# bwfbowen/muax

Hardware: AMD Instinct MI355X
Metric: batched act() env-steps/sec at num_simulations=50 (higher is better)
Workload: dtype f32; 1 GPU; cartpole: 4096 roots/GPU, obs 4, MLP embed 8, A=2, support 10, num_simulations=50, dirichlet 0.25/0.3, tiebreak=threefry, temperature 1; roots_per_gpu=4096, num_simulations=50, parallelism=roots sharded x1, no collective, backend=none (one rank), launcher=none

## Files before the change

### muax_amd/csrc/mz_act.hip

```cpp
#include <hip/hip_runtime.h>

#include <cstdlib>
#include <cstring>

#include "mz_handle.h"
#include "mz_fused_launch.h"
#include "mz_wide_launch.h"

using mzh::fail;

template <class Call>
static int dispatch_with_scratch(mzs_handle* h, mz::FusedParams& p, int* rc, Call call) {
  const size_t BN = (size_t)h->cfg.batch * (h->cfg.num_simulations + 1);
  *rc = call();
  for (int tries = 0; tries < 2 && (*rc == mz::kNeedEmbScratch || *rc >= mz::kNeedPathScratch); ++tries) {
    if (*rc == mz::kNeedEmbScratch) {
      MZS_HIP(h, hipMalloc(reinterpret_cast<void**>(&h->fused_emb), BN * h->cfg.embed_dim * sizeof(float)));
      p.emb_scratch = h->fused_emb;
    } else {
      const int words = *rc - mz::kNeedPathScratch;
      if (h->fused_path) MZS_HIP(h, hipFree(h->fused_path));
      h->fused_path = nullptr;
      h->fused_path_words = 0;
      MZS_HIP(h, hipMalloc(reinterpret_cast<void**>(&h->fused_path), BN * words * sizeof(int32_t)));
      h->fused_path_words = words;
      p.path_scratch = h->fused_path;
      p.path_words = words;
    }
    *rc = call();
  }
  return MZS_OK;
}

extern "C" {

int mzs_act_mlp(mzs_handle* h, const mzs_act_args* a, void* stream_) {
  if (!h) return MZS_E_INVALID;
  if (!a || a->struct_size != (int32_t)sizeof(mzs_act_args))
    return fail(h, MZS_E_INVALID, "mzs_act_mlp: null or size mismatch (ABI)");
  if (!h->have_weights) return fail(h, MZS_E_INVALID, "mzs_act_mlp: call mzs_mlp_set_weights first");
  if (!a->obs || !a->action || !a->action_weights || !a->root_value)
    return fail(h, MZS_E_INVALID, "mzs_act_mlp: obs/action/action_weights/root_value must be set");
  const mzs_config& c = h->cfg;
  if (c.policy == 0 && !a->dirichlet_noise && a->dirichlet_fraction != 0.0f)
    return fail(h, MZS_E_INVALID, "mzs_act_mlp: dirichlet_fraction != 0 needs dirichlet_noise");
  if (c.num_simulations > mz::kMaxSims) {
    if (h->allow_generic) return mzh::act_mlp_generic(h, a, stream_);
    return fail(h, MZS_E_UNSUPPORTED, "mzs_act_mlp: no fused kernel instance for num_simulations > 256; use the generic route "
                                      "(mzs_mlp_allow_generic) or the step-wise path");
  }
  hipStream_t stream = static_cast<hipStream_t>(stream_);
  MZS_HIP(h, hipSetDevice(c.device));

  mz::FusedParams p;
  memset(&p, 0, sizeof p);
  p.obs = a->obs; p.dirichlet_noise = a->dirichlet_noise; p.invalid = a->invalid_actions; p.gumbel = a->gumbel;
  const mzs_mlp_weights& w = h->w;
  mzh::copy_weights(w, p);
  p.action = a->action; p.action_weights = a->action_weights; p.root_value = a->root_value;
  p.search_value = a->search_value; p.depth_sum = a->depth_sum;
  if (a->tree) {
    const mzs_tree_view& t = *a->tree;
    const void* const* tp = reinterpret_cast<const void* const*>(&t);
    for (int i = 0; i < 12; ++i)
      if (!tp[i]) return fail(h, MZS_E_INVALID, "mzs_act_mlp: tree view has a null array");
    p.t_node_visits = t.node_visits; p.t_raw_values = t.raw_values; p.t_node_values = t.node_values;
    p.t_parents = t.parents; p.t_action_from_parent = t.action_from_parent;
    p.t_children_index = t.children_index; p.t_children_prior_logits = t.children_prior_logits;
    p.t_children_values = t.children_values; p.t_children_visits = t.children_visits;
    p.t_children_rewards = t.children_rewards; p.t_children_discounts = t.children_discounts;
    p.t_embeddings = t.embeddings;
    p.export_tree = 1;
  }
  p.B = c.batch; p.obs_dim = w.obs_dim; p.S = c.num_simulations; p.max_depth = c.max_depth;
  p.support = w.support_size; p.pred_on_parent = w.recurrent_pred_on;
  p.pb_c_init = c.pb_c_init; p.pb_c_base = c.pb_c_base;
  p.dirichlet_fraction = a->dirichlet_fraction; p.discount = w.discount; p.temperature = a->temperature;
  p.global_batch = (uint64_t)c.global_batch; p.root_offset = (uint64_t)c.root_offset;
  p.prof = h->prof;
  p.emb_scratch = p.export_tree ? nullptr : h->fused_emb;
  if (c.policy == 1) {
    if (!h->fused_table) {
      const std::vector<int32_t> table = mzh::visit_table(c.max_num_considered_actions, c.num_simulations);
      MZS_HIP(h, hipMalloc(reinterpret_cast<void**>(&h->fused_table), table.size() * sizeof(int32_t)));
      MZS_HIP(h, hipMemcpy(h->fused_table, table.data(), table.size() * sizeof(int32_t), hipMemcpyHostToDevice));
    }
    p.visit_table = h->fused_table;
    p.max_considered = c.max_num_considered_actions;
    p.gumbel_scale = c.gumbel_scale;
    mzh::h_split(a->key, 2, 1, p.k_gumbel);
  }
  mzh::derive_keys(a->key, h->cfg.num_simulations, h->k_sample, h->sim_keys.data());
  p.k_sample[0] = h->k_sample[0]; p.k_sample[1] = h->k_sample[1];
  memcpy(p.sim_keys, h->sim_keys.data(), sizeof(uint32_t) * 2 * (size_t)c.num_simulations);

  const int A = c.num_actions, E = c.embed_dim, F = 2 * w.support_size + 1, N = c.num_simulations + 1;
  p.F = F;
  const int mode = c.policy == 1 ? (c.qtransform == 1 ? 3 : 2) : (c.tiebreak ? 1 : 0);
  std::vector<mz::FusedDispatch> groups = {mz::fused_dispatch_g0, mz::fused_dispatch_g1, mz::fused_dispatch_g2,
                                           mz::fused_dispatch_g3, mz::fused_dispatch_g4};
  mz::jit_dispatchers(mode, &groups);
  if (h->allow_generic && getenv("MZS_FORCE_GENERIC") != nullptr) return mzh::act_mlp_generic(h, a, stream_);
  for (int compact = (c.batch > 16 * h->cu_count) ? 1 : 0; compact >= 0; --compact) {
    p.path_scratch = h->fused_path;
    p.path_words = h->fused_path_words;
    for (size_t gi = 0; gi < groups.size(); ++gi) {
      std::string err;
      int rc = 0;
      auto call = [&] { return groups[gi](mode, c.device, p, stream, A, E, F, N, compact != 0, &err); };
      if (int e = dispatch_with_scratch(h, p, &rc, call)) return e;
      if (rc == mz::kNoFusedInstance) continue;
      if (rc != MZS_OK) return fail(h, rc, "mzs_act_mlp: %s", err.c_str());
      return MZS_OK;
    }
  }
  if (mode >= 2 ? h->allow_wide_gumbel : h->allow_wide) {
    std::string err;
    int rc = 0;
    auto call = [&] { return mz::wide_dispatch(mode, h->allow_wide_gumbel, c.device, p, stream, A, E, F, &err); };
    if (int e = dispatch_with_scratch(h, p, &rc, call)) return e;
    if (rc == MZS_OK) return MZS_OK;
    if (rc != mz::kNoFusedInstance) return fail(h, rc, "mzs_act_mlp: %s", err.c_str());
  }
  if (h->allow_generic) return mzh::act_mlp_generic(h, a, stream_);
  return fail(h, MZS_E_UNSUPPORTED,
              "mzs_act_mlp: no fused kernel instance for this (A, E, F, S) (muax_amd/csrc/mz_instances.def); use the step-wise path");
}

int mzs_act_mlp_host(mzs_handle* h, const mzs_act_host_args* a, void* stream_) {
  if (!h) return MZS_E_INVALID;
  if (!a || a->struct_size != (int32_t)sizeof(mzs_act_host_args))
    return fail(h, MZS_E_INVALID, "mzs_act_mlp_host: null or size mismatch (ABI)");
  if (!h->have_weights) return fail(h, MZS_E_INVALID, "mzs_act_mlp_host: call mzs_mlp_set_weights first");
  if (!a->obs || !a->action || !a->action_weights || !a->root_value)
    return fail(h, MZS_E_INVALID, "mzs_act_mlp_host: obs/action/action_weights/root_value must be set");
  const mzs_config& c = h->cfg;
  hipStream_t stream = static_cast<hipStream_t>(stream_);
  MZS_HIP(h, hipSetDevice(c.device));
  const size_t B = (size_t)c.batch, A = (size_t)c.num_actions, OD = (size_t)h->w.obs_dim;
  const size_t obs_b = B * OD * 4, noise_b = B * A * 4, inv_b = (B * A + 3) / 4 * 4, in_b = obs_b + noise_b + inv_b;
  const size_t out_b = B * (2 + A) * 4;
  if (h->host_in_bytes < in_b) {
    if (h->host_in) { hipHostFree(h->host_in); h->host_in = nullptr; }
    MZS_HIP(h, hipHostMalloc(&h->host_in, in_b, hipHostMallocDefault));
    h->host_in_bytes = in_b;
  }
  if (!h->host_out) MZS_HIP(h, hipHostMalloc(&h->host_out, out_b, hipHostMallocDefault));
  if (!h->dev_noise) MZS_HIP(h, hipMalloc(&h->dev_noise, noise_b));
  char* hin = static_cast<char*>(h->host_in);
  char* hin_dev = nullptr;
  float* hout_dev = nullptr;
  MZS_HIP(h, hipHostGetDevicePointer(reinterpret_cast<void**>(&hin_dev), h->host_in, 0));
  MZS_HIP(h, hipHostGetDevicePointer(reinterpret_cast<void**>(&hout_dev), h->host_out, 0));
  const bool muzero = c.policy == 0;
  const bool given = muzero && a->dirichlet_noise != nullptr;
  const bool draw = muzero && !given && a->draw_dirichlet != 0 && a->dirichlet_fraction != 0.0f;
  float* d_noise = static_cast<float*>(h->dev_noise);
  if (draw) {
    uint32_t kd[2];
    mzh::h_split(a->key, 3, 1, kd);
    if (int rc = mzs_dirichlet(c.device, kd, a->dirichlet_alpha, c.batch, c.num_actions, c.global_batch, c.root_offset,
                               d_noise, stream_))
      return fail(h, rc, "mzs_act_mlp_host: %s", mzs_last_error(nullptr));
  }
  memcpy(hin, a->obs, obs_b);
  if (given) memcpy(hin + obs_b, a->dirichlet_noise, noise_b);
  if (a->invalid_actions) memcpy(hin + obs_b + noise_b, a->invalid_actions, B * A);
  float* dout = hout_dev;
  mzs_act_args args;
  memset(&args, 0, sizeof args);
  args.struct_size = (int32_t)sizeof args;
  args.obs = reinterpret_cast<const float*>(hin_dev);
  args.dirichlet_noise = draw ? d_noise : (given ? reinterpret_cast<const float*>(hin_dev + obs_b) : nullptr);
  args.invalid_actions = a->invalid_actions ? reinterpret_cast<const uint8_t*>(hin_dev + obs_b + noise_b) : nullptr;
  args.key[0] = a->key[0]; args.key[1] = a->key[1];
  args.dirichlet_fraction = (given || draw) ? a->dirichlet_fraction : 0.0f;
  args.temperature = a->temperature;
  args.action = reinterpret_cast<int32_t*>(dout);
  args.action_weights = dout + B;
  args.root_value = dout + B + B * A;
  if (int rc = mzs_act_mlp(h, &args, stream_)) return rc;
  MZS_HIP(h, hipStreamSynchronize(stream));
  const char* hout = static_cast<const char*>(h->host_out);
  memcpy(a->action, hout, B * 4);
  memcpy(a->action_weights, hout + B * 4, B * A * 4);
  memcpy(a->root_value, hout + B * 4 + B * A * 4, B * 4);
  return MZS_OK;
}

#ifdef MZ_PROFILE
int mzs_debug_profile(mzs_handle* h, uint64_t* device_buffer) {
  if (!h) return MZS_E_INVALID;
  h->prof = device_buffer;
  return MZS_OK;
}
#endif

}
```

### muax_amd/csrc/mz_api.hip

```cpp
#include <hip/hip_runtime.h>

#include <cstdio>
#include <cstring>
#include <mutex>

#include "mz_handle.h"
#include "mz_fused_launch.h"

namespace {

thread_local std::string g_create_error;

std::mutex g_jit_mutex;
std::vector<mz::FusedDispatch> g_jit_dispatch;
std::vector<mz::FusedDispatch> g_jit_dispatch_muzero;
struct JitTrain { int A, E, F; mzh::JitTrainLaunch launch; };
std::vector<JitTrain> g_jit_train;
struct JitStochTrain { int A, C, E, F, OB; mzh::JitTrainLaunch launch; };
std::vector<JitStochTrain> g_jit_stoch_train;

}

int mzh::fail(mzs_handle* h, int code, const char* fmt, const char* a) {
  char buf[512];
  snprintf(buf, sizeof buf, fmt, a);
  if (h) h->err = buf; else g_create_error = buf;
  return code;
}
mzh::JitTrainLaunch mzh::jit_train_instance(int A, int E, int F) {
  std::lock_guard<std::mutex> lock(g_jit_mutex);
  for (const JitTrain& t : g_jit_train)
    if (t.A == A && t.E == E && t.F == F) return t.launch;
  return nullptr;
}
mzh::JitTrainLaunch mzh::jit_stochastic_train_instance(int A, int C, int E, int F, int obs_dim) {
  std::lock_guard<std::mutex> lock(g_jit_mutex);
  const JitStochTrain* best = nullptr;
  for (const JitStochTrain& t : g_jit_stoch_train)
    if (t.A == A && t.C == C && t.E == E && t.F == F && obs_dim >= 1 && obs_dim <= t.OB && (!best || t.OB < best->OB)) best = &t;
  return best ? best->launch : nullptr;
}
void mz::jit_dispatchers(int mode, std::vector<FusedDispatch>* out) {
  std::lock_guard<std::mutex> lock(g_jit_mutex);
  if (mode < 2) out->insert(out->end(), g_jit_dispatch_muzero.begin(), g_jit_dispatch_muzero.end());
  out->insert(out->end(), g_jit_dispatch.begin(), g_jit_dispatch.end());
}
using mzh::fail;

extern "C" {

int mzs_abi_version(void) { return MZS_ABI_VERSION; }
int mzs_fused_jit_abi(void) { return MZS_ABI_VERSION * 1000 + (int)(sizeof(mz::FusedParams) % 1000); }

int mzs_register_train_dispatch(void* launch, int32_t num_actions, int32_t embed_dim, int32_t full_support, int32_t jit_abi) {
  if (!launch) return fail(nullptr, MZS_E_INVALID, "mzs_register_train_dispatch: null");
  if (jit_abi != mzs_train_jit_abi())
    return fail(nullptr, MZS_E_INVALID, "mzs_register_train_dispatch: the side library was built from other sources (ABI)");
  std::lock_guard<std::mutex> lock(g_jit_mutex);
  for (const JitTrain& t : g_jit_train)
    if (t.A == num_actions && t.E == embed_dim && t.F == full_support) return MZS_OK;
  g_jit_train.push_back({num_actions, embed_dim, full_support, reinterpret_cast<mzh::JitTrainLaunch>(launch)});
  return MZS_OK;
}

int mzs_register_stochastic_train_dispatch(void* launch, int32_t num_actions, int32_t num_chance_outcomes, int32_t embed_dim,
                                           int32_t full_support, int32_t obs_cap, int32_t jit_abi) {
  if (!launch) return fail(nullptr, MZS_E_INVALID, "mzs_register_stochastic_train_dispatch: null");
  if (jit_abi != mzs_stochastic_train_jit_abi())
    return fail(nullptr, MZS_E_INVALID,
                "mzs_register_stochastic_train_dispatch: the side library was built from other sources (ABI)");
  if (obs_cap != 32 && obs_cap != 64 && obs_cap != 96 && obs_cap != 128)
    return fail(nullptr, MZS_E_INVALID, "mzs_register_stochastic_train_dispatch: obs_cap must be 32, 64, 96 or 128");
  std::lock_guard<std::mutex> lock(g_jit_mutex);
  for (const JitStochTrain& t : g_jit_stoch_train)
    if (t.A == num_actions && t.C == num_chance_outcomes && t.E == embed_dim && t.F == full_support && t.OB == obs_cap)
      return MZS_OK;
  g_jit_stoch_train.push_back({num_actions, num_chance_outcomes, embed_dim, full_support, obs_cap,
                               reinterpret_cast<mzh::JitTrainLaunch>(launch)});
  return MZS_OK;
}

const char* mzs_last_error(const mzs_handle* h) { return h ? h->err.c_str() : g_create_error.c_str(); }

int mzs_create(const mzs_config* cfg, mzs_handle** out) {
  if (!cfg || !out) return fail(nullptr, MZS_E_INVALID, "mzs_create: null argument");
  if (cfg->struct_size != (int32_t)sizeof(mzs_config))
    return fail(nullptr, MZS_E_INVALID, "mzs_create: mzs_config size mismatch (ABI)");
  if (cfg->batch <= 0 || cfg->num_actions <= 0 || cfg->num_simulations <= 0 || cfg->embed_dim <= 0)
    return fail(nullptr, MZS_E_INVALID, "mzs_create: batch, num_actions, num_simulations, embed_dim must be positive");
  if (cfg->num_actions > 64) return fail(nullptr, MZS_E_UNSUPPORTED, "mzs_create: num_actions > 64");
  if (cfg->num_simulations >= 65535) return fail(nullptr, MZS_E_UNSUPPORTED, "mzs_create: num_simulations too large");
  if (cfg->policy < 0 || cfg->policy > 2)
    return fail(nullptr, MZS_E_INVALID, "mzs_create: policy must be 0 (muzero), 1 (gumbel) or 2 (stochastic)");
  if (cfg->policy == 2) {
    const int es = cfg->state_embed_dim > 0 ? cfg->state_embed_dim : cfg->embed_dim;
    const int ea = cfg->afterstate_embed_dim > 0 ? cfg->afterstate_embed_dim : cfg->embed_dim;
    if (cfg->num_chance_outcomes <= 0) return fail(nullptr, MZS_E_INVALID, "mzs_create: the stochastic policy needs num_chance_outcomes > 0");
    if (cfg->num_actions + cfg->num_chance_outcomes > 64)
      return fail(nullptr, MZS_E_UNSUPPORTED, "mzs_create: num_actions + num_chance_outcomes > 64");
    if (cfg->embed_dim != (es > ea ? es : ea))
      return fail(nullptr, MZS_E_INVALID, "mzs_create: embed_dim must be max(state_embed_dim, afterstate_embed_dim)");
    if (cfg->embed_dim >= mz::kWideEmb)
      return fail(nullptr, MZS_E_UNSUPPORTED, "mzs_create: the stochastic policy takes embeddings narrower than 256 floats");
    static_assert(mz::kWideEmb == 256, "the message above names the bound");
  } else if (cfg->num_chance_outcomes != 0) {
    return fail(nullptr, MZS_E_INVALID, "mzs_create: num_chance_outcomes is for policy 2 (stochastic) only");
  }
  if (cfg->qtransform != 0 && !(cfg->qtransform == 1 && cfg->policy == 1))
    return fail(nullptr, MZS_E_UNSUPPORTED, "mzs_create: qtransform_completed_by_mix_value is built for the gumbel policy only");
  if (cfg->policy == 1 && cfg->max_num_considered_actions < 0)
    return fail(nullptr, MZS_E_INVALID, "mzs_create: max_num_considered_actions");
  if (int rc = mzh::check_device(cfg->device, "mzs_create")) return rc;
  hipDeviceProp_t prop;
  if (hipGetDeviceProperties(&prop, cfg->device) != hipSuccess)
    return fail(nullptr, MZS_E_RUNTIME, "mzs_create: hipGetDeviceProperties failed");
  if (strncmp(prop.gcnArchName, "gfx950", 6) != 0)
    return fail(nullptr, MZS_E_NODEVICE, "mzs_create: device is %s, kernels are built for gfx950 only", prop.gcnArchName);
  mzs_handle* h = new mzs_handle();
  h->cfg = *cfg;
  h->cu_count = prop.multiProcessorCount;
  if (h->cfg.global_batch <= 0) h->cfg.global_batch = cfg->batch;
  if (h->cfg.state_embed_dim <= 0) h->cfg.state_embed_dim = cfg->embed_dim;
  if (h->cfg.afterstate_embed_dim <= 0) h->cfg.afterstate_embed_dim = cfg->embed_dim;
  if (h->cfg.root_offset < 0 || h->cfg.root_offset + cfg->batch > h->cfg.global_batch) {
    delete h;
    return fail(nullptr, MZS_E_INVALID, "mzs_create: root_offset + batch exceeds global_batch");
  }
  memset(&h->w, 0, sizeof h->w);
  h->sim_keys.assign(2 * (size_t)cfg->num_simulations, 0u);
  *out = h;
  return MZS_OK;
}

int mzs_mlp_allow_generic(mzs_handle* h, int32_t allow) {
  if (!h) return MZS_E_INVALID;
  h->allow_generic = allow != 0;
  return MZS_OK;
}
int mzs_mlp_allow_wide(mzs_handle* h, int32_t allow) {
  if (!h) return MZS_E_INVALID;
  h->allow_wide = allow != 0;
  return MZS_OK;
}
int mzs_mlp_allow_wide_gumbel(mzs_handle* h, int32_t allow) {
  if (!h) return MZS_E_INVALID;
  h->allow_wide_gumbel = allow != 0;
  return MZS_OK;
}

int mzs_destroy(mzs_handle* h) {
  if (!h) return MZS_OK;
  hipSetDevice(h->cfg.device);
  h->step.release();
  if (h->fused_table) hipFree(h->fused_table);
  if (h->fused_emb) hipFree(h->fused_emb);
  if (h->fused_path) hipFree(h->fused_path);
  if (h->jump_slab) hipFree(h->jump_slab);
  if (h->host_in) hipHostFree(h->host_in);
  if (h->host_out) hipHostFree(h->host_out);
  if (h->dev_noise) hipFree(h->dev_noise);
  if (h->gen_scratch) hipFree(h->gen_scratch);
  delete h;
  return MZS_OK;
}

int mzs_mlp_set_weights(mzs_handle* h, const mzs_mlp_weights* w) {
  if (!h) return MZS_E_INVALID;
  if (!w || w->struct_size != (int32_t)sizeof(mzs_mlp_weights))
    return fail(h, MZS_E_INVALID, "mzs_mlp_set_weights: null or size mismatch (ABI)");
  if (h->cfg.policy == 2)
    return fail(h, MZS_E_UNSUPPORTED, "mzs_mlp_set_weights: a stochastic handle runs the step-wise *_stochastic entries only");
  const float* const* ptrs = &w->repr_w;
  for (int i = 0; i < 18; ++i)
    if (!ptrs[i]) return fail(h, MZS_E_INVALID, "mzs_mlp_set_weights: null weight pointer");
  if (w->obs_dim <= 0 || w->support_size <= 0) return fail(h, MZS_E_INVALID, "mzs_mlp_set_weights: obs_dim/support_size");
  h->w = *w;
  h->have_weights = true;
  return MZS_OK;
}

static int register_dispatch(std::vector<mz::FusedDispatch>& list, void* dispatch, int32_t jit_abi) {
  if (!dispatch) return fail(nullptr, MZS_E_INVALID, "mzs_register_fused_dispatch: null");
  if (jit_abi != mzs_fused_jit_abi()) return fail(nullptr, MZS_E_INVALID, "mzs_register_fused_dispatch: the side library was built from other sources (ABI)");
  std::lock_guard<std::mutex> lock(g_jit_mutex);
  for (auto f : list)
    if (reinterpret_cast<void*>(f) == dispatch) return MZS_OK;
  list.push_back(reinterpret_cast<mz::FusedDispatch>(dispatch));
  return MZS_OK;
}
int mzs_register_fused_dispatch(void* dispatch, int32_t jit_abi) { return register_dispatch(g_jit_dispatch, dispatch, jit_abi); }
int mzs_register_fused_dispatch_muzero(void* dispatch, int32_t jit_abi) {
  return register_dispatch(g_jit_dispatch_muzero, dispatch, jit_abi);
}

}
```

### muax_amd/csrc/mz_fused_launch.h

```cpp
#pragma once
#include <string>
#include <vector>

#include "mz_fused.cuh"

namespace mz {
constexpr int kNoFusedInstance = 1;
constexpr int kNeedPathScratch = 1000;
constexpr int kNeedEmbScratch = 2;
using FusedDispatch = int (*)(int mode, int device, const FusedParams& p, hipStream_t stream, int A, int E, int F,
                              int N, bool compact, std::string* err);
int fused_dispatch_g0(int mode, int device, const FusedParams& p, hipStream_t stream, int A, int E, int F, int N, bool compact, std::string* err);
int fused_dispatch_g1(int mode, int device, const FusedParams& p, hipStream_t stream, int A, int E, int F, int N, bool compact, std::string* err);
int fused_dispatch_g2(int mode, int device, const FusedParams& p, hipStream_t stream, int A, int E, int F, int N, bool compact, std::string* err);
int fused_dispatch_g3(int mode, int device, const FusedParams& p, hipStream_t stream, int A, int E, int F, int N, bool compact, std::string* err);
int fused_dispatch_g4(int mode, int device, const FusedParams& p, hipStream_t stream, int A, int E, int F, int N, bool compact, std::string* err);
void jit_dispatchers(int mode, std::vector<FusedDispatch>* out);
}
```

### muax_amd/csrc/mz_handle.h

```cpp
#pragma once
#include <string>
#include <vector>

#include "mz_host.h"
#include "mz_keys.h"
#include "mz_step_jump.cuh"

struct mzs_handle {
  mzs_config cfg;
  std::string err;
  bool have_weights = false;
  mzs_mlp_weights w;
  mz::StepState step;
  uint32_t k_sample[2] = {0, 0};
  std::vector<uint32_t> sim_keys;
  uint64_t* prof = nullptr;
  int32_t* fused_table = nullptr;
  float* fused_emb = nullptr;
  int32_t* fused_path = nullptr;
  int fused_path_words = 0;
  int cu_count = 0;
  void* host_in = nullptr; void* host_out = nullptr; void* dev_noise = nullptr;
  size_t host_in_bytes = 0;
  mz::JumpArgs jump = {nullptr, nullptr, nullptr, nullptr};
  void* jump_slab = nullptr;
  bool use_jump = false;
  int jump_roots = 0;
  bool allow_generic = false;
  float* gen_scratch = nullptr;
  bool allow_wide = false;
  bool allow_wide_gumbel = false;
  bool have_stochastic_weights = false;
  mzs_stochastic_mlp_weights sw = {};
  int32_t stoch_obs_dim = 0;
  const float *stoch_repr_w = nullptr, *stoch_repr_b = nullptr;
};

namespace mzh {

int act_mlp_generic(mzs_handle* h, const mzs_act_args* a, void* stream);

}
```

### muax_amd/csrc/mz_keys.h

```cpp
#pragma once
#include <cstddef>
#include <cstdint>
#include <vector>

namespace mzh {

inline uint32_t rotl32(uint32_t x, int r) { return (x << r) | (x >> (32 - r)); }
inline void h_threefry(const uint32_t key[2], uint32_t x0, uint32_t x1, uint32_t out[2]) {
  static const int R[2][4] = {{13, 15, 26, 6}, {17, 29, 16, 24}};
  const uint32_t ks[3] = {key[0], key[1], key[0] ^ key[1] ^ 0x1BD11BDAu};
  x0 += ks[0];
  x1 += ks[1];
  for (int g = 0; g < 5; ++g) {
    for (int i = 0; i < 4; ++i) {
      x0 += x1;
      x1 = rotl32(x1, R[g & 1][i]) ^ x0;
    }
    x0 += ks[(g + 1) % 3];
    x1 += ks[(g + 2) % 3] + (uint32_t)(g + 1);
  }
  out[0] = x0;
  out[1] = x1;
}
inline uint32_t h_bits(const uint32_t key[2], uint64_t size, uint64_t i) {
  uint64_t half = (size + 1) / 2;
  uint64_t blk = i < half ? i : i - half;
  uint64_t c1 = half + blk;
  uint32_t out[2];
  h_threefry(key, (uint32_t)blk, c1 < size ? (uint32_t)c1 : 0u, out);
  return i < half ? out[0] : out[1];
}
inline void h_split(const uint32_t key[2], uint64_t n, uint64_t row, uint32_t out[2]) {
  out[0] = h_bits(key, 2 * n, 2 * row);
  out[1] = h_bits(key, 2 * n, 2 * row + 1);
}

inline void considered_visits(int m, int S, int32_t* seq) {
  if (m <= 1) {
    for (int i = 0; i < S; ++i) seq[i] = i;
    return;
  }
  int log2max = 0;
  while ((1 << log2max) < m) ++log2max;
  std::vector<int32_t> visits(m, 0);
  int n = 0, nc = m;
  while (n < S) {
    int extra = S / (log2max * nc);
    if (extra < 1) extra = 1;
    for (int e = 0; e < extra; ++e) {
      for (int i = 0; i < nc && n < S; ++i) seq[n++] = visits[i];
      for (int i = 0; i < nc; ++i) visits[i] += 1;
    }
    nc = nc / 2 > 2 ? nc / 2 : 2;
  }
}
inline std::vector<int32_t> visit_table(int max_considered, int S) {
  std::vector<int32_t> table((size_t)(max_considered + 1) * S);
  for (int m = 0; m <= max_considered; ++m) considered_visits(m, S, table.data() + (size_t)m * S);
  return table;
}

inline void derive_keys(const uint32_t key[2], int S, uint32_t k_sample[2], uint32_t* sim_keys) {
  uint32_t rk[2];
  h_split(key, 3, 0, k_sample);
  h_split(key, 3, 2, rk);
  for (int s = 0; s < S; ++s) {
    uint32_t nk[2];
    h_split(rk, 3, 1, &sim_keys[2 * (size_t)s]);
    h_split(rk, 3, 0, nk);
    rk[0] = nk[0], rk[1] = nk[1];
  }
}

}
```

Measured before the change: 35.46 million env-steps/s.

## Cache act dispatch plan and params block, dedupe threefry key derivation

Keeps a per-handle plan holding the resolved dispatch function, the compact/wide choice and a prefilled FusedParams block. Later act calls only patch the per-call fields and jump straight to the cached dispatcher, skipping the group-vector rebuild and probing. Key derivation now computes one split-by-3 threefry batch per step and writes simulation keys directly into the params block, removing redundant hashing and a memcpy. The plan is invalidated on weight, flag, profile or JIT-registration changes, which adds state that could go stale if another setting changes without an invalidation. Optional host timing marks are also added behind a compile flag.

```diff
diff --git a/muax_amd/csrc/mz_act.hip b/muax_amd/csrc/mz_act.hip
--- a/muax_amd/csrc/mz_act.hip
+++ b/muax_amd/csrc/mz_act.hip
@@ -8,12 +8,26 @@
 #include "mz_wide_launch.h"
 
 using mzh::fail;
+
+#ifdef MZ_HOST_TIMING
+#include <time.h>
+static thread_local int64_t g_host_marks[8];
+static inline int64_t host_now_ns() {
+  timespec ts;
+  clock_gettime(CLOCK_MONOTONIC, &ts);
+  return (int64_t)ts.tv_sec * 1000000000LL + ts.tv_nsec;
+}
+#define MZ_HT(i) (g_host_marks[i] = host_now_ns())
+#else
+#define MZ_HT(i) ((void)0)
+#endif
 
 template <class Call>
 static int dispatch_with_scratch(mzs_handle* h, mz::FusedParams& p, int* rc, Call call) {
   const size_t BN = (size_t)h->cfg.batch * (h->cfg.num_simulations + 1);
   *rc = call();
   for (int tries = 0; tries < 2 && (*rc == mz::kNeedEmbScratch || *rc >= mz::kNeedPathScratch); ++tries) {
+    h->act_plan.valid = false;
     if (*rc == mz::kNeedEmbScratch) {
       MZS_HIP(h, hipMalloc(reinterpret_cast<void**>(&h->fused_emb), BN * h->cfg.embed_dim * sizeof(float)));
       p.emb_scratch = h->fused_emb;
@@ -32,9 +46,58 @@
   return MZS_OK;
 }
 
-extern "C" {
-
-int mzs_act_mlp(mzs_handle* h, const mzs_act_args* a, void* stream_) {
+static void act_fill_handle_fields(const mzs_handle* h, mz::FusedParams& p) {
+  const mzs_config& c = h->cfg;
+  const mzs_mlp_weights& w = h->w;
+  memset(&p, 0, sizeof p);
+  mzh::copy_weights(w, p);
+  p.B = c.batch; p.obs_dim = w.obs_dim; p.S = c.num_simulations; p.max_depth = c.max_depth;
+  p.support = w.support_size; p.F = 2 * w.support_size + 1; p.pred_on_parent = w.recurrent_pred_on;
+  p.pb_c_init = c.pb_c_init; p.pb_c_base = c.pb_c_base;
+  p.discount = w.discount;
+  p.global_batch = (uint64_t)c.global_batch; p.root_offset = (uint64_t)c.root_offset;
+  p.prof = h->prof;
+  if (c.policy == 1) {
+    p.visit_table = h->fused_table;
+    p.max_considered = c.max_num_considered_actions;
+    p.gumbel_scale = c.gumbel_scale;
+  }
+}
+
+static bool act_patch_call(const mzs_handle* h, const mzs_act_args* a, mz::FusedParams& p) {
+  p.obs = a->obs; p.dirichlet_noise = a->dirichlet_noise; p.invalid = a->invalid_actions; p.gumbel = a->gumbel;
+  p.action = a->action; p.action_weights = a->action_weights; p.root_value = a->root_value;
+  p.search_value = a->search_value; p.depth_sum = a->depth_sum;
+  if (a->tree) {
+    const mzs_tree_view& t = *a->tree;
+    const void* const* tp = reinterpret_cast<const void* const*>(&t);
+    for (int i = 0; i < 12; ++i)
+      if (!tp[i]) return false;
+    p.t_node_visits = t.node_visits; p.t_raw_values = t.raw_values; p.t_node_values = t.node_values;
+    p.t_parents = t.parents; p.t_action_from_parent = t.action_from_parent;
+    p.t_children_index = t.children_index; p.t_children_prior_logits = t.children_prior_logits;
+    p.t_children_values = t.children_values; p.t_children_visits = t.children_visits;
+    p.t_children_rewards = t.children_rewards; p.t_children_discounts = t.children_discounts;
+    p.t_embeddings = t.embeddings;
+    p.export_tree = 1;
+  } else if (p.export_tree) {
+    p.t_node_visits = nullptr; p.t_raw_values = nullptr; p.t_node_values = nullptr;
+    p.t_parents = nullptr; p.t_action_from_parent = nullptr;
+    p.t_children_index = nullptr; p.t_children_prior_logits = nullptr;
+    p.t_children_values = nullptr; p.t_children_visits = nullptr;
+    p.t_children_rewards = nullptr; p.t_children_discounts = nullptr;
+    p.t_embeddings = nullptr;
+    p.export_tree = 0;
+  }
+  p.dirichlet_fraction = a->dirichlet_fraction; p.temperature = a->temperature;
+  p.emb_scratch = p.export_tree ? nullptr : h->fused_emb;
+  p.path_scratch = h->fused_path;
+  p.path_words = h->fused_path_words;
+  if (h->cfg.policy == 1) mzh::h_split(a->key, 2, 1, p.k_gumbel);
+  return true;
+}
+
+static int act_mlp(mzs_handle* h, const mzs_act_args* a, void* stream_) {
   if (!h) return MZS_E_INVALID;
   if (!a || a->struct_size != (int32_t)sizeof(mzs_act_args))
     return fail(h, MZS_E_INVALID, "mzs_act_mlp: null or size mismatch (ABI)");
@@ -51,66 +114,68 @@
   }
   hipStream_t stream = static_cast<hipStream_t>(stream_);
   MZS_HIP(h, hipSetDevice(c.device));
-
-  mz::FusedParams p;
-  memset(&p, 0, sizeof p);
-  p.obs = a->obs; p.dirichlet_noise = a->dirichlet_noise; p.invalid = a->invalid_actions; p.gumbel = a->gumbel;
-  const mzs_mlp_weights& w = h->w;
-  mzh::copy_weights(w, p);
-  p.action = a->action; p.action_weights = a->action_weights; p.root_value = a->root_value;
-  p.search_value = a->search_value; p.depth_sum = a->depth_sum;
-  if (a->tree) {
-    const mzs_tree_view& t = *a->tree;
-    const void* const* tp = reinterpret_cast<const void* const*>(&t);
-    for (int i = 0; i < 12; ++i)
-      if (!tp[i]) return fail(h, MZS_E_INVALID, "mzs_act_mlp: tree view has a null array");
-    p.t_node_visits = t.node_visits; p.t_raw_values = t.raw_values; p.t_node_values = t.node_values;
-    p.t_parents = t.parents; p.t_action_from_parent = t.action_from_parent;
-    p.t_children_index = t.children_index; p.t_children_prior_logits = t.children_prior_logits;
-    p.t_children_values = t.children_values; p.t_children_visits = t.children_visits;
-    p.t_children_rewards = t.children_rewards; p.t_children_discounts = t.children_discounts;
-    p.t_embeddings = t.embeddings;
-    p.export_tree = 1;
-  }
-  p.B = c.batch; p.obs_dim = w.obs_dim; p.S = c.num_simulations; p.max_depth = c.max_depth;
-  p.support = w.support_size; p.pred_on_parent = w.recurrent_pred_on;
-  p.pb_c_init = c.pb_c_init; p.pb_c_base = c.pb_c_base;
-  p.dirichlet_fraction = a->dirichlet_fraction; p.discount = w.discount; p.temperature = a->temperature;
-  p.global_batch = (uint64_t)c.global_batch; p.root_offset = (uint64_t)c.root_offset;
-  p.prof = h->prof;
-  p.emb_scratch = p.export_tree ? nullptr : h->fused_emb;
-  if (c.policy == 1) {
-    if (!h->fused_table) {
-      const std::vector<int32_t> table = mzh::visit_table(c.max_num_considered_actions, c.num_simulations);
-      MZS_HIP(h, hipMalloc(reinterpret_cast<void**>(&h->fused_table), table.size() * sizeof(int32_t)));
-      MZS_HIP(h, hipMemcpy(h->fused_table, table.data(), table.size() * sizeof(int32_t), hipMemcpyHostToDevice));
-    }
+  MZ_HT(1);
+
+  mz::ActPlan& plan = h->act_plan;
+  mz::FusedParams& p = plan.block;
+  const uint64_t generation = mz::jit_generation();
+  if (plan.valid && plan.generation != generation) plan.valid = false;
+  const bool planned = plan.valid;
+  if (!planned) act_fill_handle_fields(h, p);
+  if (!act_patch_call(h, a, p)) return fail(h, MZS_E_INVALID, "mzs_act_mlp: tree view has a null array");
+  if (c.policy == 1 && !h->fused_table) {
+    const std::vector<int32_t> table = mzh::visit_table(c.max_num_considered_actions, c.num_simulations);
+    MZS_HIP(h, hipMalloc(reinterpret_cast<void**>(&h->fused_table), table.size() * sizeof(int32_t)));
+    MZS_HIP(h, hipMemcpy(h->fused_table, table.data(), table.size() * sizeof(int32_t), hipMemcpyHostToDevice));
     p.visit_table = h->fused_table;
-    p.max_considered = c.max_num_considered_actions;
-    p.gumbel_scale = c.gumbel_scale;
-    mzh::h_split(a->key, 2, 1, p.k_gumbel);
-  }
-  mzh::derive_keys(a->key, h->cfg.num_simulations, h->k_sample, h->sim_keys.data());
-  p.k_sample[0] = h->k_sample[0]; p.k_sample[1] = h->k_sample[1];
-  memcpy(p.sim_keys, h->sim_keys.data(), sizeof(uint32_t) * 2 * (size_t)c.num_simulations);
-
-  const int A = c.num_actions, E = c.embed_dim, F = 2 * w.support_size + 1, N = c.num_simulations + 1;
-  p.F = F;
+  }
+  MZ_HT(2);
+  mzh::derive_keys(a->key, c.num_simulations, p.k_sample, &p.sim_keys[0][0]);
+  h->k_sample[0] = p.k_sample[0]; h->k_sample[1] = p.k_sample[1];
+  MZ_HT(3);
+
+  const int A = c.num_actions, E = c.embed_dim, F = p.F, N = c.num_simulations + 1;
   const int mode = c.policy == 1 ? (c.qtransform == 1 ? 3 : 2) : (c.tiebreak ? 1 : 0);
+  if (planned) {
+    std::string err;
+    int rc = 0;
+    const mz::FusedDispatch dispatch = plan.dispatch;
+    const bool wide = plan.wide, compact = plan.compact;
+    auto call = [&] {
+      return wide ? mz::wide_dispatch(mode, h->allow_wide_gumbel, c.device, p, stream, A, E, F, &err)
+                  : dispatch(mode, c.device, p, stream, A, E, F, N, compact, &err);
+    };
+    MZ_HT(4);
+    if (int e = dispatch_with_scratch(h, p, &rc, call)) return e;
+    MZ_HT(5);
+    if (rc == MZS_OK) {
+      plan.valid = true;
+      return MZS_OK;
+    }
+    plan.valid = false;
+    if (rc != mz::kNoFusedInstance) return fail(h, rc, "mzs_act_mlp: %s", err.c_str());
+  }
+  plan.valid = false;
+  auto keep = [&](mz::FusedDispatch dispatch, bool wide, bool compact) {
+    plan.dispatch = dispatch; plan.wide = wide; plan.compact = compact;
+    plan.generation = generation;
+    plan.valid = true;
+  };
   std::vector<mz::FusedDispatch> groups = {mz::fused_dispatch_g0, mz::fused_dispatch_g1, mz::fused_dispatch_g2,
                                            mz::fused_dispatch_g3, mz::fused_dispatch_g4};
   mz::jit_dispatchers(mode, &groups);
   if (h->allow_generic && getenv("MZS_FORCE_GENERIC") != nullptr) return mzh::act_mlp_generic(h, a, stream_);
   for (int compact = (c.batch > 16 * h->cu_count) ? 1 : 0; compact >= 0; --compact) {
-    p.path_scratch = h->fused_path;
-    p.path_words = h->fused_path_words;
     for (size_t gi = 0; gi < groups.size(); ++gi) {
       std::string err;
       int rc = 0;
       auto call = [&] { return groups[gi](mode, c.device, p, stream, A, E, F, N, compact != 0, &err); };
+      MZ_HT(4);
       if (int e = dispatch_with_scratch(h, p, &rc, call)) return e;
+      MZ_HT(5);
       if (rc == mz::kNoFusedInstance) continue;
       if (rc != MZS_OK) return fail(h, rc, "mzs_act_mlp: %s", err.c_str());
+      keep(groups[gi], false, compact != 0);
       return MZS_OK;
     }
   }
@@ -118,13 +183,27 @@
     std::string err;
     int rc = 0;
     auto call = [&] { return mz::wide_dispatch(mode, h->allow_wide_gumbel, c.device, p, stream, A, E, F, &err); };
+    MZ_HT(4);
     if (int e = dispatch_with_scratch(h, p, &rc, call)) return e;
-    if (rc == MZS_OK) return MZS_OK;
+    MZ_HT(5);
+    if (rc == MZS_OK) {
+      keep(nullptr, true, false);
+      return MZS_OK;
+    }
     if (rc != mz::kNoFusedInstance) return fail(h, rc, "mzs_act_mlp: %s", err.c_str());
   }
   if (h->allow_generic) return mzh::act_mlp_generic(h, a, stream_);
   return fail(h, MZS_E_UNSUPPORTED,
               "mzs_act_mlp: no fused kernel instance for this (A, E, F, S) (muax_amd/csrc/mz_instances.def); use the step-wise path");
+}
+
+extern "C" {
+
+int mzs_act_mlp(mzs_handle* h, const mzs_act_args* a, void* stream_) {
+  MZ_HT(0);
+  const int rc = act_mlp(h, a, stream_);
+  MZ_HT(6);
+  return rc;
 }
 
 int mzs_act_mlp_host(mzs_handle* h, const mzs_act_host_args* a, void* stream_) {
@@ -188,10 +267,18 @@
   return MZS_OK;
 }
 
+#ifdef MZ_HOST_TIMING
+int mzs_debug_host_timing(int64_t* out) {
+  memcpy(out, g_host_marks, sizeof g_host_marks);
+  return MZS_OK;
+}
+#endif
+
 #ifdef MZ_PROFILE
 int mzs_debug_profile(mzs_handle* h, uint64_t* device_buffer) {
   if (!h) return MZS_E_INVALID;
   h->prof = device_buffer;
+  h->act_plan.valid = false;
   return MZS_OK;
 }
 #endif
diff --git a/muax_amd/csrc/mz_api.hip b/muax_amd/csrc/mz_api.hip
--- a/muax_amd/csrc/mz_api.hip
+++ b/muax_amd/csrc/mz_api.hip
@@ -1,6 +1,7 @@
 #include <hip/hip_runtime.h>
 
 #include <cstdio>
+#include <atomic>
 #include <cstring>
 #include <mutex>
 
@@ -14,6 +15,7 @@
 std::mutex g_jit_mutex;
 std::vector<mz::FusedDispatch> g_jit_dispatch;
 std::vector<mz::FusedDispatch> g_jit_dispatch_muzero;
+std::atomic<uint64_t> g_jit_generation{0};
 struct JitTrain { int A, E, F; mzh::JitTrainLaunch launch; };
 std::vector<JitTrain> g_jit_train;
 struct JitStochTrain { int A, C, E, F, OB; mzh::JitTrainLaunch launch; };
@@ -45,6 +47,7 @@
   if (mode < 2) out->insert(out->end(), g_jit_dispatch_muzero.begin(), g_jit_dispatch_muzero.end());
   out->insert(out->end(), g_jit_dispatch.begin(), g_jit_dispatch.end());
 }
+uint64_t mz::jit_generation() { return g_jit_generation.load(std::memory_order_acquire); }
 using mzh::fail;
 
 extern "C" {
@@ -135,16 +138,19 @@
 int mzs_mlp_allow_generic(mzs_handle* h, int32_t allow) {
   if (!h) return MZS_E_INVALID;
   h->allow_generic = allow != 0;
+  h->act_plan.valid = false;
   return MZS_OK;
 }
 int mzs_mlp_allow_wide(mzs_handle* h, int32_t allow) {
   if (!h) return MZS_E_INVALID;
   h->allow_wide = allow != 0;
+  h->act_plan.valid = false;
   return MZS_OK;
 }
 int mzs_mlp_allow_wide_gumbel(mzs_handle* h, int32_t allow) {
   if (!h) return MZS_E_INVALID;
   h->allow_wide_gumbel = allow != 0;
+  h->act_plan.valid = false;
   return MZS_OK;
 }
 
@@ -176,6 +182,7 @@
   if (w->obs_dim <= 0 || w->support_size <= 0) return fail(h, MZS_E_INVALID, "mzs_mlp_set_weights: obs_dim/support_size");
   h->w = *w;
   h->have_weights = true;
+  h->act_plan.valid = false;
   return MZS_OK;
 }
 
@@ -186,6 +193,7 @@
   for (auto f : list)
     if (reinterpret_cast<void*>(f) == dispatch) return MZS_OK;
   list.push_back(reinterpret_cast<mz::FusedDispatch>(dispatch));
+  g_jit_generation.fetch_add(1, std::memory_order_release);
   return MZS_OK;
 }
 int mzs_register_fused_dispatch(void* dispatch, int32_t jit_abi) { return register_dispatch(g_jit_dispatch, dispatch, jit_abi); }
diff --git a/muax_amd/csrc/mz_fused_launch.h b/muax_amd/csrc/mz_fused_launch.h
--- a/muax_amd/csrc/mz_fused_launch.h
+++ b/muax_amd/csrc/mz_fused_launch.h
@@ -16,4 +16,5 @@
 int fused_dispatch_g3(int mode, int device, const FusedParams& p, hipStream_t stream, int A, int E, int F, int N, bool compact, std::string* err);
 int fused_dispatch_g4(int mode, int device, const FusedParams& p, hipStream_t stream, int A, int E, int F, int N, bool compact, std::string* err);
 void jit_dispatchers(int mode, std::vector<FusedDispatch>* out);
+uint64_t jit_generation();
 }
diff --git a/muax_amd/csrc/mz_handle.h b/muax_amd/csrc/mz_handle.h
--- a/muax_amd/csrc/mz_handle.h
+++ b/muax_amd/csrc/mz_handle.h
@@ -2,9 +2,21 @@
 #include <string>
 #include <vector>
 
+#include "mz_fused_launch.h"
 #include "mz_host.h"
 #include "mz_keys.h"
 #include "mz_step_jump.cuh"
+
+namespace mz {
+struct ActPlan {
+  bool valid = false;
+  bool wide = false;
+  bool compact = false;
+  FusedDispatch dispatch = nullptr;
+  uint64_t generation = 0;
+  FusedParams block;
+};
+}
 
 struct mzs_handle {
   mzs_config cfg;
@@ -20,6 +32,7 @@
   int32_t* fused_path = nullptr;
   int fused_path_words = 0;
   int cu_count = 0;
+  mz::ActPlan act_plan;
   void* host_in = nullptr; void* host_out = nullptr; void* dev_noise = nullptr;
   size_t host_in_bytes = 0;
   mz::JumpArgs jump = {nullptr, nullptr, nullptr, nullptr};
diff --git a/muax_amd/csrc/mz_keys.h b/muax_amd/csrc/mz_keys.h
--- a/muax_amd/csrc/mz_keys.h
+++ b/muax_amd/csrc/mz_keys.h
@@ -60,15 +60,23 @@
   return table;
 }
 
+__attribute__((always_inline)) inline void h_split3(const uint32_t key[2], uint32_t w[6]) {
+  uint32_t a[2], b[2], c[2];
+  h_threefry(key, 0u, 3u, a);
+  h_threefry(key, 1u, 4u, b);
+  h_threefry(key, 2u, 5u, c);
+  w[0] = a[0]; w[1] = b[0]; w[2] = c[0]; w[3] = a[1]; w[4] = b[1]; w[5] = c[1];
+}
+
 inline void derive_keys(const uint32_t key[2], int S, uint32_t k_sample[2], uint32_t* sim_keys) {
-  uint32_t rk[2];
-  h_split(key, 3, 0, k_sample);
-  h_split(key, 3, 2, rk);
+  uint32_t w[6];
+  h_split3(key, w);
+  k_sample[0] = w[0], k_sample[1] = w[1];
+  uint32_t rk[2] = {w[4], w[5]};
   for (int s = 0; s < S; ++s) {
-    uint32_t nk[2];
-    h_split(rk, 3, 1, &sim_keys[2 * (size_t)s]);
-    h_split(rk, 3, 0, nk);
-    rk[0] = nk[0], rk[1] = nk[1];
+    h_split3(rk, w);
+    sim_keys[2 * (size_t)s] = w[2], sim_keys[2 * (size_t)s + 1] = w[3];
+    rk[0] = w[0], rk[1] = w[1];
   }
 }
 
```

Measured after the change: 35.89 million env-steps/s, median of 6. No clear change (+1.2%).
